# Abolfazlmsl/Oriented-Object-Detection

Measured on AMD Instinct MI355X. Metric: 416px tiles/sec (whole node), YOLOv11n-OBB 3ch, higher is better.
Workload: dtype f32; 1 GPU; YOLOv11n-OBB 3ch 416x416 tiled inference, single-scale (BASELINE configs[1]): forward + decode + ProbIoU NMS + border filter + per-tile merge + final polygon-IoU merge; step_pipelining=True, nc=12, weights=synthetic seeded, cls bias -8 (no checkpoint offline), final_detections=12170

## Files before the change

### include/obbhip.h

```cpp
#ifndef OBBHIP_H
#define OBBHIP_H

#include <stddef.h>
#include <stdint.h>

#ifdef __cplusplus
extern "C" {
#endif

#define OBB_OK 0
#define OBB_ERR_INVALID (-1)
#define OBB_ERR_HIP (-2)
#define OBB_ERR_STATE (-3)
#define OBB_ERR_FORMAT (-4)

typedef struct obb_ctx obb_ctx;
typedef void *obb_stream_t;

int obb_version(void);
int obb_ctx_create(int device, obb_ctx **out);
int obb_ctx_destroy(obb_ctx *ctx);
const char *obb_last_error(const obb_ctx *ctx);

int obb_set_option(obb_ctx *ctx, const char *key, int64_t value);
// ... 110 lines not shown
                      int32_t B, int32_t N, int32_t nh, uint16_t *dqkv, obb_stream_t s);
int obb_add_bf16(obb_ctx *ctx, const uint16_t *a, const uint16_t *b, int64_t n, uint16_t *out, obb_stream_t s);
int obb_chanwin_bf16(obb_ctx *ctx, const uint16_t *src, int32_t Cs, int32_t s0, const uint16_t *add, int32_t Ca, int32_t a0, int64_t npix, int32_t n,
                     uint16_t *dst, int32_t Cd, int32_t d0, obb_stream_t s);

int obb_model_load(obb_ctx *ctx, const void *blob_host, size_t bytes);
int obb_model_unload(obb_ctx *ctx, int32_t slot);
int obb_model_info(const obb_ctx *ctx, int32_t h, int32_t w, int32_t *nc, int32_t *ch, int32_t *anchors, int32_t *nconv);
int obb_forward(obb_ctx *ctx, const uint8_t *tiles, int32_t B, int32_t h, int32_t w, float *head, obb_stream_t s);
int obb_forward_gate(obb_ctx *ctx, const uint8_t *tiles, int32_t B, int32_t h, int32_t w, float *head, float *cmax, obb_stream_t s);
int obb_debug_plan(obb_ctx *ctx, int32_t h, int32_t w, char *buf_host, int64_t buf_bytes, int64_t *needed);
int obb_debug_pack_1x1(int32_t form, const float *w, int32_t cout, int32_t cin, int32_t c0, int32_t nc, float *out, int64_t max_floats,
                       int64_t *needed, int32_t *tiling_host);
int obb_debug_activation(obb_ctx *ctx, int32_t h, int32_t w, int32_t B, const char *name, float *out, int64_t max_elems,
                         int64_t *n_elems, int32_t *shape_hwc_host, obb_stream_t s);
int obb_decode_nms(obb_ctx *ctx, const float *head, int32_t B, int32_t h, int32_t w, float conf_thres, float iou_thres,
                   int32_t max_det, float *out, int32_t *count, obb_stream_t s);
int obb_decode_nms_gate(obb_ctx *ctx, const float *head, const float *cmax, int32_t B, int32_t h, int32_t w, float conf_thres, float iou_thres,
                        int32_t max_det, float *det, int32_t *count, obb_stream_t s);
int obb_decode_nms_full(obb_ctx *ctx, const float *head, int32_t B, int32_t h, int32_t w, float conf_thres, float iou_thres,
                        int32_t max_det, float *out, int32_t *count, obb_stream_t s);
int obb_decode(obb_ctx *ctx, const float *head, int32_t B, int32_t h, int32_t w, float *pred, obb_stream_t s);
int obb_probiou_nms(obb_ctx *ctx, const float *boxes, const float *scores, int64_t n, float iou_thres, int32_t *order,
                    uint8_t *keep, obb_stream_t s);
int obb_results(obb_ctx *ctx, const float *det, const float *lb, int64_t n, float *xywhr, float *pts, obb_stream_t s);

int obb_probiou_loss(obb_ctx *ctx, const float *pred, const float *target, const float *weight, int64_t n, float target_scores_sum,
                     float *loss, float *grad_pred, obb_stream_t s);

int obb_tile_labels(obb_ctx *ctx, const double *labels, int64_t n, const int32_t *rects, int32_t ntiles, double min_fraction, uint8_t *mask,
// ... 66 lines not shown
```

### oriented-object-detection_amd/_lib.py

```python
import ctypes as C
import os

_HERE = os.path.dirname(os.path.abspath(__file__))
SO_PATH = os.path.join(_HERE, "libobbhip.so")
if os.environ.get("OBB_LIB"):
    import sys
    SO_PATH = os.environ["OBB_LIB"]
    sys.stderr.write("oriented_object_detection_amd: OBB_LIB is set -- loading the DIAGNOSTIC library %s instead of the product build\n" % SO_PATH)
_lib = None

c_dp, c_fp, c_ip, c_lp, c_bp = (C.POINTER(C.c_double), C.POINTER(C.c_float), C.POINTER(C.c_int32),
                                C.POINTER(C.c_int64), C.POINTER(C.c_uint8))
_V = C.c_void_p

SIGNATURES = {
    "obb_version": [],
    "obb_ctx_create": [C.c_int, C.POINTER(_V)],
    "obb_ctx_destroy": [_V],
    "obb_last_error": [_V],
    "obb_set_option": [_V, C.c_char_p, C.c_int64],
    "obb_poly_iou_pairs": [_V, _V, _V, C.c_int64, _V, _V],
    "obb_poly_iou_matrix": [_V, _V, _V, C.c_int64, _V, _V, C.c_int64, _V, _V],
    "obb_points_in_quads": [_V, _V, _V, C.c_int64, _V, _V, C.c_int64, _V, _V],
    "obb_build_multich": [_V, _V, C.c_int32, C.c_int32, C.c_int32, _V, _V],
# ... 47 lines not shown
    "obb_attn_fwd_bf16": [_V, _V, C.c_int32, C.c_int32, C.c_int32, _V, _V, _V],
    "obb_attn_bwd_bf16": [_V, _V, _V, _V, _V, _V, C.c_int32, C.c_int32, C.c_int32, _V, _V],
    "obb_add_bf16": [_V, _V, _V, C.c_int64, _V, _V],
    "obb_chanwin_bf16": [_V, _V, C.c_int32, C.c_int32, _V, C.c_int32, C.c_int32, C.c_int64, C.c_int32, _V, C.c_int32, C.c_int32, _V],
    "obb_gather_tiles": [_V, _V, C.c_int32, C.c_int32, C.c_int32, _V, C.c_int32, C.c_int32, _V, _V],
    "obb_letterbox": [_V, _V, C.c_int32, C.c_int32, C.c_int32, C.c_int32, C.c_int32, C.c_int32, C.c_int32, C.c_int32, _V,
                      C.c_int32, C.c_int32, _V],
    "obb_model_load": [_V, _V, C.c_size_t],
    "obb_model_unload": [_V, C.c_int32],
    "obb_model_info": [_V, C.c_int32, C.c_int32, c_ip, c_ip, c_ip, c_ip],
    "obb_forward": [_V, _V, C.c_int32, C.c_int32, C.c_int32, _V, _V],
    "obb_forward_gate": [_V, _V, C.c_int32, C.c_int32, C.c_int32, _V, _V, _V],
    "obb_debug_plan": [_V, C.c_int32, C.c_int32, C.c_char_p, C.c_int64, c_lp],
    "obb_debug_pack_1x1": [C.c_int32, _V, C.c_int32, C.c_int32, C.c_int32, C.c_int32, _V, C.c_int64, c_lp, c_ip],
    "obb_debug_activation": [_V, C.c_int32, C.c_int32, C.c_int32, C.c_char_p, _V, C.c_int64, c_lp, c_ip, _V],
    "obb_decode_nms": [_V, _V, C.c_int32, C.c_int32, C.c_int32, C.c_float, C.c_float, C.c_int32, _V, _V, _V],
    "obb_decode_nms_gate": [_V, _V, _V, C.c_int32, C.c_int32, C.c_int32, C.c_float, C.c_float, C.c_int32, _V, _V, _V],
    "obb_decode_nms_full": [_V, _V, C.c_int32, C.c_int32, C.c_int32, C.c_float, C.c_float, C.c_int32, _V, _V, _V],
    "obb_decode": [_V, _V, C.c_int32, C.c_int32, C.c_int32, _V, _V],
    "obb_probiou_nms": [_V, _V, _V, C.c_int64, C.c_float, _V, _V, _V],
    "obb_results": [_V, _V, _V, C.c_int64, _V, _V, _V],
    "obb_probiou_loss": [_V, _V, _V, _V, C.c_int64, C.c_float, _V, _V, _V],
    "obb_tile_labels": [_V, _V, C.c_int64, _V, C.c_int32, C.c_double, _V, _V, _V],
    "obb_dfl_loss": [_V, _V, _V, _V, C.c_int64, C.c_int32, C.c_float, _V, _V, _V],
    "obb_bce_loss": [_V, _V, _V, C.c_int64, C.c_float, _V, _V, _V],
    "obb_crit_decode": [_V, _V, C.c_int32, _V, _V, c_ip, c_ip, C.c_int32, C.c_int32, _V, _V, _V, _V, _V],
    "obb_crit_loss": [_V, _V, C.c_int32, _V, _V, c_ip, c_ip, C.c_int32, C.c_int32, _V, _V, _V, c_fp, _V, _V, _V, _V, _V, _V],
    "obb_sgd_step": [_V, _V, _V, _V, C.c_int64, C.c_float, C.c_float, C.c_float, C.c_int32, C.c_int32, _V],
    "obb_adamw_step": [_V, _V, _V, _V, _V, C.c_int64, C.c_int64, C.c_float, C.c_double, C.c_double, C.c_float, C.c_float, _V],
    "obb_grad_sumsq_partials": [c_lp, C.c_int32, c_lp],
# ... 51 lines not shown
```

### oriented-object-detection_amd/csrc/c3k2f32.h

```cpp
#pragma once
#include <hip/hip_runtime.h>

#include <vector>

#include "conv.h"

namespace obb {

struct C3k2F32Launch {
    TensorRef cat;
    TensorRef out;
    const float *w1 = nullptr, *w2 = nullptr, *wc = nullptr;
    const float *b1 = nullptr, *b2 = nullptr, *bc = nullptr;
    int B = 0, H = 0, W = 0, C = 16, CO = 64;
};

bool c3k2f32_supported(int C, int CO, int H, int W);
std::vector<int> c3k2f32_cout_perm(int CO);
void c3k2f32_tile(int H, int W, int &TH, int &TW);
hipError_t launch_c3k2f32(const C3k2F32Launch &L, hipStream_t st);

}
```

### oriented-object-detection_amd/csrc/c3k2f32.hip

```cpp
#include "c3k2f32.h"
#include "launchcfg.h"

#include <algorithm>

namespace obb {

typedef __attribute__((ext_vector_type(4))) float f32x4;
typedef __attribute__((ext_vector_type(4))) unsigned int u32x4;

struct C3k2Params {
    const float *cat; int64_t cat_bs; int cat_cs, cat_co; unsigned cat_span;
    float *out; int64_t out_bs; int out_cs, out_co, out_blk, out_ps;
    const float *wall, *b1, *b2;
    int H, W, TH, TW, tiles_x, tiles_y;
    float inv_xw, inv_tw2, inv_tw;
};

__device__ __forceinline__ float silu32c(float x) { return x * __builtin_amdgcn_rcpf(1.0f + __expf(-x)); }

constexpr int kC3MaxX = 448, kC3MaxT = 324;

template <int C, int CO>
__global__ __launch_bounds__(512, 4) void k_c3k2_f32(const C3k2Params P) {
    extern __shared__ __attribute__((aligned(16))) char smem[];
    constexpr int NT = 512, CH = C / 2, PSTX = C * 4 + 16, PSTT = CH * 4 + 16;
    constexpr int CPK1 = C / 4, KP1 = 9 * CPK1 / 4, CPK2 = CH / 4, KP2 = (9 * CPK2) / 4, KR2 = (9 * CPK2) % 4, KPC = 3 * C / 16, NFC = CO / 16;
    static_assert((9 * CPK1) % 4 == 0, "conv 1: whole pieces only");
    constexpr int XOFF = 0, TOFF = kC3MaxX * PSTX, W1OFF = TOFF + kC3MaxT * PSTT, W2OFF = W1OFF + KP1 * 1024, WCOFF = W2OFF + KP2 * 1024 + KR2 * 256,
                  BCOFF = WCOFF + NFC * KPC * 1024, NWCH = (BCOFF + CO * 4 - W1OFF) / 16;
    constexpr int F1 = 3, F2 = 2;
    constexpr unsigned NOPIX = 0xffffffffu;
    const int tid = threadIdx.x, lane = tid & 63, wave = __builtin_amdgcn_readfirstlane(tid >> 6), g = lane >> 4, pl = lane & 15;
    const int t = blockIdx.x, tx_i = t % P.tiles_x, r_ = t / P.tiles_x, ty_i = r_ % P.tiles_y, b = r_ / P.tiles_y;
    const int oy0 = ty_i * P.TH, ox0 = tx_i * P.TW;
    const int XW = P.TW + 4, XH = P.TH + 4, TW2 = P.TW + 2, TH2 = P.TH + 2;
    const int npix1 = TH2 * TW2, npix2 = P.TH * P.TW;

    const __amdgpu_buffer_rsrc_t cat_rsrc = __builtin_amdgcn_make_buffer_rsrc((void *)(P.cat + (int64_t)b * P.cat_bs + P.cat_co), 0, (int)P.cat_span, 0x00020000);
    const __amdgpu_buffer_rsrc_t w_rsrc = __builtin_amdgcn_make_buffer_rsrc((void *)P.wall, 0, NWCH * 16, 0x00020000);
    constexpr int MAXLD = (kC3MaxX * CPK1 + NT - 1) / NT, MAXW = (NWCH + NT - 1) / NT;
    u32x4 xr[MAXLD], wr[MAXW];
    const int nchunkX = XH * XW * CPK1;
#pragma unroll
    for (int k = 0; k < MAXLD; ++k) {
        const int idx = tid + k * NT, pix = idx / CPK1, c = idx - pix * CPK1;
        const int iy = (int)(((float)pix + 0.5f) * P.inv_xw), ix = pix - iy * XW;
        const int gy = oy0 - 2 + iy, gx = ox0 - 2 + ix;
        const bool ok = idx < nchunkX && gy >= 0 && gy < P.H && gx >= 0 && gx < P.W;
        xr[k] = __builtin_amdgcn_raw_buffer_load_b128(cat_rsrc, ok ? (unsigned)((((int64_t)gy * P.W + gx) * P.cat_cs + C + c * 4) * 4) : NOPIX, 0, 0);
    }
#pragma unroll
// ... 22 lines not shown
    for (int k = 0; k < MAXW; ++k) {
        const int idx = tid + k * NT;
        if (idx < NWCH) *reinterpret_cast<u32x4 *>(smem + W1OFF + idx * 16) = wr[k];
    }
    __syncthreads();

    {
        int xb[F1];
        bool val[F1];
#pragma unroll
        for (int i = 0; i < F1; ++i) {
            const int f = wave + 8 * i;
            val[i] = f < nfrag1;
            const int p = min(f * 16 + pl, npix1 - 1);
            const int r = (int)(((float)p + 0.5f) * P.inv_tw2), x = p - r * TW2;
            xb[i] = (r * XW + x) * PSTX;
        }
        f32x4 acc[F1];
#pragma unroll
        for (int i = 0; i < F1; ++i) acc[i] = f32x4{0.f, 0.f, 0.f, 0.f};
        for (int piece = 0; piece < KP1; ++piece) {
            const f32x4 w = *reinterpret_cast<const f32x4 *>(smem + W1OFF + piece * 1024 + lane * 16);
            const int q = piece * 4 + g, tap = q / CPK1, c0 = q - tap * CPK1, dy = (tap * 11) >> 5, dx = tap - dy * 3;
            const int off = (dy * XW + dx) * PSTX + c0 * 16;
            f32x4 a[F1];
#pragma unroll
            for (int i = 0; i < F1; ++i) a[i] = *reinterpret_cast<const f32x4 *>(smem + XOFF + xb[i] + off);
#pragma unroll
            for (int s = 0; s < 4; ++s)
#pragma unroll
                for (int i = 0; i < F1; ++i)
                    if (val[i]) acc[i] = __builtin_amdgcn_mfma_f32_16x16x4f32(w[s], a[i][s], acc[i], 0, 0, 0);
        }
        const float4 bv = *reinterpret_cast<const float4 *>(P.b1 + 4 * g);
#pragma unroll
        for (int i = 0; i < F1; ++i) {
            const int p = (wave + 8 * i) * 16 + pl;
            if (!val[i] || p >= npix1 || 4 * g >= CH) continue;
            const int r = (int)(((float)p + 0.5f) * P.inv_tw2), x = p - r * TW2;
            const int gy = oy0 - 1 + r, gx = ox0 - 1 + x;
            const bool inside = gy >= 0 && gy < P.H && gx >= 0 && gx < P.W;
            float4 o = make_float4(0.f, 0.f, 0.f, 0.f);
            if (inside) o = make_float4(silu32c(acc[i][0] + bv.x), silu32c(acc[i][1] + bv.y), silu32c(acc[i][2] + bv.z), silu32c(acc[i][3] + bv.w));
            *reinterpret_cast<float4 *>(smem + TOFF + (r * TW2 + x) * PSTT + g * 16) = o;
        }
    }
    __syncthreads();

    bool val2[F2];
#pragma unroll
    for (int i = 0; i < F2; ++i) val2[i] = wave + 8 * i < nfrag2;
    f32x4 acc2[F2];
#pragma unroll
    for (int i = 0; i < F2; ++i) acc2[i] = f32x4{0.f, 0.f, 0.f, 0.f};
#pragma unroll
    for (int piece = 0; piece < KP2; ++piece) {
        const f32x4 w = *reinterpret_cast<const f32x4 *>(smem + W2OFF + piece * 1024 + lane * 16);
        const int q = piece * 4 + g, tap = q / CPK2, c0 = q - tap * CPK2, dy = (tap * 11) >> 5, dx = tap - dy * 3;
        const int off = (dy * TW2 + dx) * PSTT + c0 * 16;
// ... 51 lines not shown
#pragma unroll
    for (int i = 0; i < F2; ++i) {
        if (!val2[i] || opix[i] < 0) continue;
        const int ca = P.out_co + 16 * g;
        float *op = P.out + (int64_t)b * P.out_bs + (int64_t)opix[i] * P.out_cs + (P.out_blk ? (int64_t)(ca >> 3) * P.out_ps + (ca & 7) : (int64_t)ca);
#pragma unroll
        for (int nf = 0; nf < NFC; ++nf) {
            const float4 bv = *reinterpret_cast<const float4 *>(smem + BCOFF + (nf * 16 + 4 * g) * 4);
            const float4 o = make_float4(silu32c(acc3[i][nf][0] + bv.x), silu32c(acc3[i][nf][1] + bv.y), silu32c(acc3[i][nf][2] + bv.z), silu32c(acc3[i][nf][3] + bv.w));
            float *o4 = P.out_blk ? op + (int64_t)(nf >> 1) * P.out_ps + 4 * (nf & 1) : op + 4 * nf;
            *reinterpret_cast<float4 *>(o4) = o;
        }
    }
}

void c3k2f32_tile(int H, int W, int &TH, int &TW) {
    TW = std::min(W, 52);
    if (W > 52 && W % 52 && W % 2 == 0 && W / 2 <= 52) TW = W / 2;
    int th = 1;
    while (th + 1 <= H && (th + 5) * (TW + 4) <= kC3MaxX && (th + 3) * (TW + 2) <= kC3MaxT && (th + 3) * (TW + 2) <= 24 * 16 && (th + 1) * TW <= 16 * 16) ++th;
    TH = th;
}

bool c3k2f32_supported(int C, int CO, int H, int W) {
    if (C != 16 || CO != 64 || H < 1 || W < 1) return false;
    int TH, TW;
    c3k2f32_tile(H, W, TH, TW);
    return (TH + 4) * (TW + 4) <= kC3MaxX && (TH + 2) * (TW + 2) <= kC3MaxT && (TH + 2) * (TW + 2) <= 24 * 16 && TH * TW <= 16 * 16;
}

std::vector<int> c3k2f32_cout_perm(int CO) {
    std::vector<int> p(CO);
    for (int f = 0; f < CO / 16; ++f)
        for (int r = 0; r < 16; ++r) p[16 * f + r] = 16 * (r >> 2) + 4 * f + (r & 3);
    return p;
}

hipError_t launch_c3k2f32(const C3k2F32Launch &L, hipStream_t st) {
    if (!c3k2f32_supported(L.C, L.CO, L.H, L.W) || L.cat.cpb || (L.cat.cs & 3) || (L.cat.co & 3) || !L.w1 || !L.b1 || !L.b2 || L.B < 1) return hipErrorInvalidValue;
    if (L.out.cpb && !(L.out.cpb == 2 && L.out.cs == 8 && L.out.co % 8 == 0 && L.out.ps > 0)) return hipErrorInvalidValue;
    if (!L.out.cpb && ((L.out.cs | L.out.co) & 3)) return hipErrorInvalidValue;
    C3k2Params P;
    P.cat = (const float *)L.cat.p; P.cat_bs = L.cat.bs; P.cat_cs = L.cat.cs; P.cat_co = L.cat.co;
    const int64_t span = ((int64_t)L.H * L.W * L.cat.cs - L.cat.co) * 4;
    if (span <= 0 || span >= (1ll << 32) - 65536) return hipErrorInvalidValue;
    P.cat_span = (unsigned)span;
    P.out = (float *)L.out.p; P.out_bs = L.out.bs; P.out_cs = L.out.cs; P.out_co = L.out.co; P.out_blk = L.out.cpb ? 1 : 0; P.out_ps = (int)L.out.ps;
    P.wall = L.w1; P.b1 = L.b1; P.b2 = L.b2;
    P.H = L.H; P.W = L.W;
    c3k2f32_tile(L.H, L.W, P.TH, P.TW);
    P.tiles_x = (L.W + P.TW - 1) / P.TW; P.tiles_y = (L.H + P.TH - 1) / P.TH;
    P.inv_xw = 1.0f / (float)(P.TW + 4); P.inv_tw2 = 1.0f / (float)(P.TW + 2); P.inv_tw = 1.0f / (float)P.TW;
    const int64_t ntiles = (int64_t)L.B * P.tiles_y * P.tiles_x;
    if (ntiles >= (1ll << 31)) return hipErrorInvalidValue;
    constexpr int C = 16, CO = 64;
    constexpr size_t lds = (size_t)kC3MaxX * (C * 4 + 16) + (size_t)kC3MaxT * (C / 2 * 4 + 16) + 9 * 1024 + (4 * 1024 + 2 * 256) + (CO / 16) * 3 * 1024 + CO * 4;
    hipError_t e = allow_dyn_lds((const void *)k_c3k2_f32<16, 64>, 80 * 1024);
    if (e != hipSuccess) return e;
    hipLaunchKernelGGL((k_c3k2_f32<16, 64>), dim3((unsigned)ntiles), dim3(512), lds, st, P);
    return hipGetLastError();
}

}
```

### oriented-object-detection_amd/csrc/ctx.h

```cpp
#pragma once
#include <hip/hip_runtime.h>

#include <cstdarg>
#include <cstdint>
#include <cstdio>
#include <map>
#include <memory>
#include <string>
#include <vector>

#include "../../include/obbhip.h"

namespace obb {
struct Model;
struct EngineOpts {
    bool tail = true, tail16 = true, bneck = true, bneck_cv2 = true, c3kimg = true, dwpw = true, upfold = true, stem = true, front = true, pair = true, hmerge = true,
         sppf_fuse = true, attn_mfma = true, xtile = true, nitile = true, nc2 = true, blk32 = true, c3k2f = true, pw32 = true, upacc = true, graph = true;
    int fwd_split = 0 , microbatch = 1024;
};
}

struct obb_ctx {
    int device = 0;
    std::string err;
    struct Slot { void *p = nullptr; size_t bytes = 0; };
    std::vector<Slot> ws;
    std::shared_ptr<obb::Model> model;
    std::map<int, std::shared_ptr<obb::Model>> slots;
    int slot = 0;
    bool opt_f16 = true;
    bool opt_f32 = false;
    obb::EngineOpts opt;
// ... 28 lines not shown
```

### oriented-object-detection_amd/csrc/engine.hip

```cpp
#include <algorithm>
#include <cmath>
#include <cstdlib>
#include <cstring>

#include "plan.h"

namespace obb {

static int ensure_capacity(obb_ctx *ctx, Plan &P, int B) {
    if (B <= P.cap) return OBB_OK;
    int cap = std::max(B, 1);
    int64_t off = 0;
    for (Buf &b : P.bufs) {
        b.off = off;
        if (b.virt) continue;
        off += ((int64_t)cap * b.per_img() * (b.f32 ? 4 : 2) + 255) / 256 * 256;
    }
    void *slab = nullptr;
    OBB_HIP(ctx, hipDeviceSynchronize());
    P.drop_graphs();
    if (P.slab) { (void)hipFree(P.slab); P.slab = nullptr; P.cap = 0; }
    OBB_HIP(ctx, hipMalloc(&slab, (size_t)off + 256));
    P.slab = slab;
    P.cap = cap;
// ... 214 lines not shown
}

__global__ void k_f32_slice_copy(const float *__restrict__ src, int64_t bs, int cs, int co, int C, int64_t npix_per_img, int B, float *__restrict__ dst, int blk) {
    int64_t i = (int64_t)blockIdx.x * 256 + threadIdx.x;
    if (i >= (int64_t)B * npix_per_img * C) return;
    int c = (int)(i % C) + co;
    int64_t pix = (i / C) % npix_per_img;
    int64_t b = i / ((int64_t)C * npix_per_img);
    dst[i] = blk > 0 ? src[b * bs + (int64_t)(c / blk) * npix_per_img * blk + pix * blk + c % blk] : src[b * bs + pix * cs + c];
}

static bool *switch_of(obb_ctx *ctx, const std::string &k) {
    struct { const char *key; bool *flag; } sw[] = {
        {"tail", &ctx->opt.tail}, {"tail16", &ctx->opt.tail16}, {"bneck", &ctx->opt.bneck}, {"bneck_cv2", &ctx->opt.bneck_cv2},
        {"c3kimg", &ctx->opt.c3kimg}, {"dwpw", &ctx->opt.dwpw}, {"upfold", &ctx->opt.upfold}, {"stem", &ctx->opt.stem}, {"front", &ctx->opt.front}, {"pair", &ctx->opt.pair},
        {"hmerge", &ctx->opt.hmerge}, {"sppf_fuse", &ctx->opt.sppf_fuse}, {"attn_mfma", &ctx->opt.attn_mfma}, {"xtile", &ctx->opt.xtile}, {"nitile", &ctx->opt.nitile}, {"nc2", &ctx->opt.nc2}, {"blk32", &ctx->opt.blk32}, {"c3k2f", &ctx->opt.c3k2f}, {"pw32", &ctx->opt.pw32}, {"upacc", &ctx->opt.upacc}, {"graph", &ctx->opt.graph}};
    for (auto &e : sw)
        if (k == e.key) return e.flag;
    return nullptr;
}

}

using namespace obb;

extern "C" {

int obb_model_load(obb_ctx *ctx, const void *blob_host, size_t bytes) {
    OBB_REQUIRE(ctx, ctx && blob_host && bytes > 0, "obb_model_load: bad arguments");
    OBB_HIP(ctx, hipSetDevice(ctx->device));
    OBB_HIP(ctx, hipDeviceSynchronize());
// ... 174 lines not shown
                break;
            }
            case OP_DW: snprintf(line, sizeof line, "dwconv %s c%d out%dx%d macs%.0f\n", op.name.c_str(), op.in.C, op.Ho, op.Wo, op.macs); break;
            case OP_C3KIMG: snprintf(line, sizeof line, "c3kimg %s c%d out%dx%d macs%.0f\n", op.name.c_str(), op.in.C, op.Ho, op.Wo, op.macs); break;
            case OP_DWPW: snprintf(line, sizeof line, "dwpw %s c%d tail%d out%dx%d macs%.0f\n", op.name.c_str(), op.dwpw.cin, op.dwpw.tail_cout, op.Ho, op.Wo, op.macs); break;
            case OP_BNECK: snprintf(line, sizeof line, "bneck %s c%d co%d out%dx%d rows4 macs%.0f\n", op.name.c_str(), op.bneck.C, op.bneck.CO, op.Ho, op.Wo, op.macs); break;
            case OP_SPPF: snprintf(line, sizeof line, "pool %s c%d out%dx%d x3 macs0\n", op.name.c_str(), op.in.C, op.Ho, op.Wo); break;
            case OP_POOL: snprintf(line, sizeof line, "pool %s c%d out%dx%d macs0\n", op.name.c_str(), op.in.C, op.Ho, op.Wo); break;
            case OP_UP: snprintf(line, sizeof line, "upsample %s c%d out%dx%d macs0\n", op.name.c_str(), op.in.C, op.Ho, op.Wo); break;
            case OP_PW32:
                snprintf(line, sizeof line, "pw32 %s k1 s1 cin%d cout%d out%dx%d waves%d raw%d lds%d macs%.0f\n", op.name.c_str(), op.pw32.cin, op.pw32.cout, op.Ho, op.Wo,
                         op.pw32.cin * 256 <= 80 * 1024 ? 8 : 16, op.pw32.raw ? 1 : 0, op.pw32.cin * 256, op.macs);
                break;
            case OP_C3K2F32: {
                int th, tw;
                c3k2f32_tile(op.H, op.W, th, tw);
                snprintf(line, sizeof line, "c3k2f32 %s c%d co%d out%dx%d TH%d TW%d macs%.0f\n", op.name.c_str(), op.c3k2f.C, op.c3k2f.CO, op.Ho, op.Wo, th, tw, op.macs);
                break;
            }
            case OP_STEM32:
                snprintf(line, sizeof line, "stem32 %s k3 s2 cin%d cout%d out%dx%d rows%d macs%.0f\n", op.name.c_str(), op.stem32.cin, op.stem32.cout, op.Ho, op.Wo, 4, op.macs);
                break;
            case OP_STEM:
                snprintf(line, sizeof line, "stem %s k3 s2 cin%d cout%d out%dx%d rows%d macs%.0f\n", op.name.c_str(), op.stem.cin, op.stem.cout, op.Ho, op.Wo, 4, op.macs);
                break;
            case OP_FRONT: snprintf(line, sizeof line, "front %s cin%d out%dx%d macs%.0f\n", op.name.c_str(), op.front.cin, op.Ho, op.Wo, op.macs); break;
            case OP_ATTN: snprintf(line, sizeof line, "attn %s N%d nh%d macs%.0f\n", op.name.c_str(), op.N, op.nh, op.macs); break;
        }
        out += line;
    }
    snprintf(line, sizeof line, "total_macs %.0f bytes_per_img %lld nbufs %zu nops %zu\n", P->macs_per_img, (long long)P->bytes_per_img, P->bufs.size(),
             P->ops.size());
// ... 22 lines not shown
    const int64_t hw = (int64_t)b.H * b.W;
    const int64_t d_bs = b.blk > 0 ? hw * b.blk : b.per_img(), d_ps = b.blk > 0 ? (int64_t)P->cap * hw * b.blk : 0;
    if (b.f32)
        hipLaunchKernelGGL(k_f32_slice_copy, dim3((unsigned)cdiv(n, 256)), dim3(256), 0, (hipStream_t)s, (const float *)b.p, (int64_t)b.per_img(), b.C, sl.co, sl.C, hw,
                           B, out, b.blk32);
    else if (ctx->model->f16)
        hipLaunchKernelGGL(k_half_slice_to_f32<true>, dim3((unsigned)cdiv(n, 256)), dim3(256), 0, (hipStream_t)s, (const bf16_t *)b.p, d_bs, b.C,
                           sl.co, sl.C, hw, B, out, b.blk, d_ps);
    else
        hipLaunchKernelGGL(k_half_slice_to_f32<false>, dim3((unsigned)cdiv(n, 256)), dim3(256), 0, (hipStream_t)s, (const bf16_t *)b.p, d_bs, b.C,
                           sl.co, sl.C, hw, B, out, b.blk, d_ps);
    OBB_LAUNCH_CHECK(ctx);
    return OBB_OK;
}

}
```

### oriented-object-detection_amd/csrc/netplan.hip

```cpp
#include <algorithm>
#include <cmath>
#include <cstring>

#include "plan.h"

namespace obb {

#pragma pack(push, 1)
struct BlobHeader { char magic[4]; uint32_t version, nrec; int32_t nc, ch; float width, depth; int32_t max_ch, reg_max; char scale[8]; };
struct BlobRec { char name[64]; int32_t c1, c2, k, s, g, act; uint64_t w_off, b_off; };
#pragma pack(pop)

int parse_blob(obb_ctx *ctx, Model &M) {
    const size_t n = M.blob.size();
    if (n < sizeof(BlobHeader)) return set_error(ctx, OBB_ERR_FORMAT, "weight blob too small (%zu bytes)", n);
    BlobHeader H;
    memcpy(&H, M.blob.data(), sizeof H);
    if (memcmp(H.magic, "OBBW", 4) != 0 || H.version != 1) return set_error(ctx, OBB_ERR_FORMAT, "bad weight blob magic/version");
    if (H.reg_max != kRegMax) return set_error(ctx, OBB_ERR_FORMAT, "reg_max %d unsupported", H.reg_max);
    if (H.ch != 3 && H.ch != 4) return set_error(ctx, OBB_ERR_FORMAT, "input channels %d unsupported (3 or 4)", H.ch);
    if (H.nc < 1 || H.nc > 1024) return set_error(ctx, OBB_ERR_FORMAT, "nc %d out of range", H.nc);
    M.nc = H.nc; M.ch = H.ch; M.width = H.width; M.depth = H.depth; M.max_ch = H.max_ch;
    M.scale = std::string(H.scale, strnlen(H.scale, 8));
    size_t tbl = sizeof(BlobHeader);
// ... 536 lines not shown
            for (int i = 0; i < n; ++i) {
                Slice src = sub(cat, (1 + i) * c, c), dst = sub(cat, (2 + i) * c, c);
                if (use_c3k) c3k(name + ".m." + std::to_string(i), src, H, W, dst, 2);
                else bottleneck(name + ".m." + std::to_string(i), src, H, W, dst, 0.5);
            }
        }
        conv(name + ".cv2", whole(cat), H, W, out);
    }
    bool c3k2_f32(const std::string &name, int cat, int c, int H, int W, Slice out) {
        if (!M.f32 || !M.o.tail || !M.o.c3k2f || out.buf < 0 || P.bufs[out.buf].virt || P.bufs[cat].blk32 || !c3k2f32_supported(c, out.C, H, W)) return false;
        const ConvRecord *r1 = rec(name + ".m.0.cv1"), *r2 = rec(name + ".m.0.cv2"), *rc = rec(name + ".cv2");
        if (!r1 || !r2 || !rc || err) return false;
        if (!rec_is(r1, 3, c, c / 2) || !rec_is(r2, 3, c / 2, c) || !rec_is(rc, 1, 3 * c, out.C)) return false;
        const std::vector<int> perm = c3k2f32_cout_perm(out.C);
        const Conv32Tiling t1{1, 1, c, 1, 1, 1, 1}, t2{1, 1, c / 2, 1, 1, 1, 1}, tc{1, 1, 3 * c, out.C / 16, 1, 1, 1};
        std::vector<float> wall = pack_conv32_weights(r1->w, c / 2, c, 3, t1, nullptr, false);
        const std::vector<float> w2 = pack_conv32_weights(r2->w, c, c / 2, 3, t2, nullptr, false), wc = pack_conv32_weights(rc->w, out.C, 3 * c, 1, tc, perm.data(), false);
        wall.insert(wall.end(), w2.begin(), w2.end());
        wall.insert(wall.end(), wc.begin(), wc.end());
        for (int i = 0; i < out.C; ++i) wall.push_back(rc->b[perm[i]]);
        if (wall.size() != (size_t)(9 * 256 + 4 * 256 + 2 * 64 + (out.C / 16) * 3 * 256 + out.C)) { err = set_error(ctx, OBB_ERR_STATE, "c3k2 fp32 kernel: weight image has %zu floats", wall.size()); return false; }
        Op op;
        op.type = OP_C3K2F32; op.name = name + ".m.0+" + name + ".cv2"; op.in = sub(cat, 0, 2 * c); op.out = out; op.H = H; op.W = W; op.Ho = H; op.Wo = W;
        C3k2F32Launch &L = op.c3k2f;
        L.H = H; L.W = W; L.C = c; L.CO = out.C;
        L.w1 = upload(wall); L.b1 = bias_padded(r1, nullptr, 64); L.b2 = bias_padded(r2, nullptr, 64);
        op.macs = (double)H * W * (9.0 * c * (c / 2) * 2 + 3.0 * c * out.C);
        emit(op, name + ".cv2", out);
        return true;
    }

    void head_tail(const std::string &conv1, const std::string &conv2, Slice in, int level, int H, int W, int tmp, Slice head_slice) {
        if (tail_ok(conv1, conv2, H, W)) return conv(conv1, in, H, W, head_slice, Slice(), level, nullptr, conv2.c_str());
        conv(conv1, in, H, W, whole(tmp));
        conv(conv2, whole(tmp), H, W, head_slice, Slice(), level);
    }

    int build() {
        const int h = P.h, w = P.w;
        const bool big = M.scale == "m" || M.scale == "l" || M.scale == "x";
// ... 169 lines not shown
```

### oriented-object-detection_amd/ops.py

```python
import ctypes as C
import contextlib
import ctypes as _ct
import os
from typing import List, Optional

import torch

from . import _lib

_ctx = {}
T = torch.Tensor


def ctx(device=None):
    idx = torch.cuda.current_device() if device is None else torch.device(device).index or 0
    if idx not in _ctx:
        h = C.c_void_p()
        _lib.check(_lib.lib().obb_ctx_create(idx, C.byref(h)))
        _ctx[idx] = h
    return _ctx[idx]


def destroy_contexts():
    for h in _ctx.values():
# ... 1093 lines not shown
    if n:
        _O.records_to_dets(rec, n, r, int(strike_cls), gb, c, f, a)
    return gb, c, f, a


def gather_compact(recv):
    r = _chk(recv, torch.int32, "recv")
    world, cap = r.shape[0], r.shape[1] - 1
    out = torch.empty((world * cap, 12), dtype=torch.int32, device=r.device)
    counts = torch.empty(world + 1, dtype=torch.int32, device=r.device)
    _O.gather_compact(r, out, counts)
    return out, counts


PRECISIONS = {"f16": 16, "fp16": 16, "bf16": 1016, "f32": 32, "fp32": 32}
MODEL_OPTIONS = ("fuse", "tail", "tail16", "bneck", "bneck_cv2", "c3kimg", "dwpw", "upfold", "stem", "front", "pair", "hmerge", "sppf_fuse", "attn_mfma", "xtile", "nitile", "nc2", "blk32", "c3k2f", "pw32", "upacc", "graph")


def select_model(slot, device=None):
    _call("obb_set_option", ctx(device), b"model_slot", int(slot))


def get_option(key, device=None):
    v = C.c_int64(0)
    _call("obb_get_option", ctx(device), key.encode(), C.byref(v))
    return v.value


@contextlib.contextmanager
def engine_state(device=None):
    keys = ("precision",) + MODEL_OPTIONS[1:]
# ... 74 lines not shown
    c = ctx(device)
    need = C.c_int64(0)
    _call("obb_debug_plan", c, h, w, None, 0, C.byref(need))
    buf = C.create_string_buffer(need.value)
    _call("obb_debug_plan", c, h, w, buf, need.value, C.byref(need))
    return buf.value.decode().strip().split("\n")


def debug_activation(name, B, h, w, device=None):
    c = ctx(device)
    n = C.c_int64(0)
    shp = (C.c_int32 * 3)()
    _call("obb_debug_activation", c, h, w, B, name.encode(), None, 0, C.byref(n), shp, _stream())
    out = torch.empty((B, shp[0], shp[1], shp[2]), dtype=torch.float32, device=torch.device("cuda", torch.cuda.current_device()))
    _O.debug_activation(name, B, h, w, out)
    return out


def decode(head, h, w):
    hd = _padded_head(_chk(head, torch.float32, "head"))
    B, A, _ = hd.shape
    pred = torch.empty((B, A, 4 + model_info(h, w, hd.device)["nc"] + 1), dtype=torch.float32, device=hd.device)
    _O.decode(hd, h, w, pred)
    return pred


def decode_nms(head, h, w, conf=0.25, iou=0.7, max_det=300, full=False, zero=True, cmax=None):
    hd = _padded_head(_chk(head, torch.float32, "head"))
    B = hd.shape[0]
    det = (torch.zeros if zero or not B else torch.empty)((B, max_det, 7), dtype=torch.float32, device=hd.device)
# ... 462 lines not shown
```

Measured before the change: 33160 tiles/s.

## Compute two output rows per MFMA fragment in fused C3k2 fp32 first conv

The first 3x3 conv in the fused C3k2 block has only 8 output channels, so half of each 16-wide MFMA fragment was padding. A new rows form packs 8 couts x 2 adjacent output rows into the 16 fragment rows, using a 4x3 (12-tap) weight layout, so the number of fragment columns (pixels) in conv1 is roughly halved. It is enabled by default through a new c3k2rows option and requires even tile heights. A debug entry point to compare the block forms is also added. In exchange it does more K steps per fragment (12 taps instead of 9, with zero-padded weights) and may shrink or change the tile height.

```diff
diff --git a/include/obbhip.h b/include/obbhip.h
--- a/include/obbhip.h
+++ b/include/obbhip.h
@@ -148,6 +148,9 @@
                        int64_t *needed, int32_t *tiling_host);
 int obb_debug_activation(obb_ctx *ctx, int32_t h, int32_t w, int32_t B, const char *name, float *out, int64_t max_elems,
                          int64_t *n_elems, int32_t *shape_hwc_host, obb_stream_t s);
+int obb_debug_c3k2_block(obb_ctx *ctx, int32_t form, int32_t B, int32_t H, int32_t W, int32_t C, int32_t CO, const float *w1_host,
+                         const float *b1_host, const float *w2_host, const float *b2_host, const float *wc_host, const float *bc_host, float *cat3,
+                         float *tmp, float *out, obb_stream_t s);
 int obb_decode_nms(obb_ctx *ctx, const float *head, int32_t B, int32_t h, int32_t w, float conf_thres, float iou_thres,
                    int32_t max_det, float *out, int32_t *count, obb_stream_t s);
 int obb_decode_nms_gate(obb_ctx *ctx, const float *head, const float *cmax, int32_t B, int32_t h, int32_t w, float conf_thres, float iou_thres,
diff --git a/oriented-object-detection_amd/_lib.py b/oriented-object-detection_amd/_lib.py
--- a/oriented-object-detection_amd/_lib.py
+++ b/oriented-object-detection_amd/_lib.py
@@ -85,6 +85,7 @@
     "obb_debug_plan": [_V, C.c_int32, C.c_int32, C.c_char_p, C.c_int64, c_lp],
     "obb_debug_pack_1x1": [C.c_int32, _V, C.c_int32, C.c_int32, C.c_int32, C.c_int32, _V, C.c_int64, c_lp, c_ip],
     "obb_debug_activation": [_V, C.c_int32, C.c_int32, C.c_int32, C.c_char_p, _V, C.c_int64, c_lp, c_ip, _V],
+    "obb_debug_c3k2_block": [_V, C.c_int32, C.c_int32, C.c_int32, C.c_int32, C.c_int32, C.c_int32, _V, _V, _V, _V, _V, _V, _V, _V, _V, _V],
     "obb_decode_nms": [_V, _V, C.c_int32, C.c_int32, C.c_int32, C.c_float, C.c_float, C.c_int32, _V, _V, _V],
     "obb_decode_nms_gate": [_V, _V, _V, C.c_int32, C.c_int32, C.c_int32, C.c_float, C.c_float, C.c_int32, _V, _V, _V],
     "obb_decode_nms_full": [_V, _V, C.c_int32, C.c_int32, C.c_int32, C.c_float, C.c_float, C.c_int32, _V, _V, _V],
diff --git a/oriented-object-detection_amd/csrc/c3k2f32.h b/oriented-object-detection_amd/csrc/c3k2f32.h
--- a/oriented-object-detection_amd/csrc/c3k2f32.h
+++ b/oriented-object-detection_amd/csrc/c3k2f32.h
@@ -13,11 +13,13 @@
     const float *w1 = nullptr, *w2 = nullptr, *wc = nullptr;
     const float *b1 = nullptr, *b2 = nullptr, *bc = nullptr;
     int B = 0, H = 0, W = 0, C = 16, CO = 64;
+    bool rows = true;
 };
 
 bool c3k2f32_supported(int C, int CO, int H, int W);
 std::vector<int> c3k2f32_cout_perm(int CO);
-void c3k2f32_tile(int H, int W, int &TH, int &TW);
+void c3k2f32_tile(int H, int W, int &TH, int &TW, bool rows = true);
+std::vector<float> pack_c3k2_rows_weights(const float *w_oihw, int C);
 hipError_t launch_c3k2f32(const C3k2F32Launch &L, hipStream_t st);
 
 }
diff --git a/oriented-object-detection_amd/csrc/c3k2f32.hip b/oriented-object-detection_amd/csrc/c3k2f32.hip
--- a/oriented-object-detection_amd/csrc/c3k2f32.hip
+++ b/oriented-object-detection_amd/csrc/c3k2f32.hip
@@ -20,21 +20,31 @@
 
 constexpr int kC3MaxX = 448, kC3MaxT = 324;
 
-template <int C, int CO>
+template <int C, int CO, bool ROWS>
+struct C3k2Lds {
+    static constexpr int CH = C / 2, PSTX = C * 4 + 16, PSTT = CH * 4 + 16;
+    static constexpr int CPK1 = C / 4, TAPS1 = ROWS ? 12 : 9, KP1 = TAPS1 * CPK1 / 4, CPK2 = CH / 4, KP2 = (9 * CPK2) / 4, KR2 = (9 * CPK2) % 4, KPC = 3 * C / 16, NFC = CO / 16;
+    static constexpr int XOFF = 0, TOFF = kC3MaxX * PSTX, W1OFF = TOFF + kC3MaxT * PSTT, W2OFF = W1OFF + KP1 * 1024, WCOFF = W2OFF + KP2 * 1024 + KR2 * 256,
+                         BCOFF = WCOFF + NFC * KPC * 1024, BYTES = BCOFF + CO * 4, NWCH = (BYTES - W1OFF) / 16;
+    static_assert((TAPS1 * CPK1) % 4 == 0, "conv 1: whole pieces only");
+    static_assert(2 * BYTES <= 160 * 1024, "two workgroups per CU");
+};
+
+template <int C, int CO, bool ROWS>
 __global__ __launch_bounds__(512, 4) void k_c3k2_f32(const C3k2Params P) {
     extern __shared__ __attribute__((aligned(16))) char smem[];
-    constexpr int NT = 512, CH = C / 2, PSTX = C * 4 + 16, PSTT = CH * 4 + 16;
-    constexpr int CPK1 = C / 4, KP1 = 9 * CPK1 / 4, CPK2 = CH / 4, KP2 = (9 * CPK2) / 4, KR2 = (9 * CPK2) % 4, KPC = 3 * C / 16, NFC = CO / 16;
-    static_assert((9 * CPK1) % 4 == 0, "conv 1: whole pieces only");
-    constexpr int XOFF = 0, TOFF = kC3MaxX * PSTX, W1OFF = TOFF + kC3MaxT * PSTT, W2OFF = W1OFF + KP1 * 1024, WCOFF = W2OFF + KP2 * 1024 + KR2 * 256,
-                  BCOFF = WCOFF + NFC * KPC * 1024, NWCH = (BCOFF + CO * 4 - W1OFF) / 16;
-    constexpr int F1 = 3, F2 = 2;
+    using LY = C3k2Lds<C, CO, ROWS>;
+    constexpr int NT = 512, CH = LY::CH, PSTX = LY::PSTX, PSTT = LY::PSTT;
+    constexpr int CPK1 = LY::CPK1, KP1 = LY::KP1, CPK2 = LY::CPK2, KP2 = LY::KP2, KR2 = LY::KR2, KPC = LY::KPC, NFC = LY::NFC;
+    constexpr int XOFF = LY::XOFF, TOFF = LY::TOFF, W1OFF = LY::W1OFF, W2OFF = LY::W2OFF, WCOFF = LY::WCOFF, BCOFF = LY::BCOFF, NWCH = LY::NWCH;
+    static_assert(!ROWS || CH == 8, "rows form: 8 couts x 2 rows fill the fragment");
+    constexpr int F1 = ROWS ? 2 : 3, F2 = 2;
     constexpr unsigned NOPIX = 0xffffffffu;
     const int tid = threadIdx.x, lane = tid & 63, wave = __builtin_amdgcn_readfirstlane(tid >> 6), g = lane >> 4, pl = lane & 15;
     const int t = blockIdx.x, tx_i = t % P.tiles_x, r_ = t / P.tiles_x, ty_i = r_ % P.tiles_y, b = r_ / P.tiles_y;
     const int oy0 = ty_i * P.TH, ox0 = tx_i * P.TW;
     const int XW = P.TW + 4, XH = P.TH + 4, TW2 = P.TW + 2, TH2 = P.TH + 2;
-    const int npix1 = TH2 * TW2, npix2 = P.TH * P.TW;
+    const int npix1 = (ROWS ? TH2 >> 1 : TH2) * TW2, npix2 = P.TH * P.TW;
 
     const __amdgpu_buffer_rsrc_t cat_rsrc = __builtin_amdgcn_make_buffer_rsrc((void *)(P.cat + (int64_t)b * P.cat_bs + P.cat_co), 0, (int)P.cat_span, 0x00020000);
     const __amdgpu_buffer_rsrc_t w_rsrc = __builtin_amdgcn_make_buffer_rsrc((void *)P.wall, 0, NWCH * 16, 0x00020000);
@@ -87,7 +97,7 @@
             val[i] = f < nfrag1;
             const int p = min(f * 16 + pl, npix1 - 1);
             const int r = (int)(((float)p + 0.5f) * P.inv_tw2), x = p - r * TW2;
-            xb[i] = (r * XW + x) * PSTX;
+            xb[i] = ((ROWS ? 2 * r : r) * XW + x) * PSTX;
         }
         f32x4 acc[F1];
 #pragma unroll
@@ -105,17 +115,19 @@
                 for (int i = 0; i < F1; ++i)
                     if (val[i]) acc[i] = __builtin_amdgcn_mfma_f32_16x16x4f32(w[s], a[i][s], acc[i], 0, 0, 0);
         }
-        const float4 bv = *reinterpret_cast<const float4 *>(P.b1 + 4 * g);
+        const int cg = ROWS ? (g & 1) : g, dyr = ROWS ? (g >> 1) : 0;
+        const float4 bv = *reinterpret_cast<const float4 *>(P.b1 + 4 * cg);
 #pragma unroll
         for (int i = 0; i < F1; ++i) {
             const int p = (wave + 8 * i) * 16 + pl;
-            if (!val[i] || p >= npix1 || 4 * g >= CH) continue;
-            const int r = (int)(((float)p + 0.5f) * P.inv_tw2), x = p - r * TW2;
+            if (!val[i] || p >= npix1 || 4 * cg >= CH) continue;
+            const int rp = (int)(((float)p + 0.5f) * P.inv_tw2), x = p - rp * TW2, r = ROWS ? 2 * rp + dyr : rp;
+            if (r >= TH2) continue;
             const int gy = oy0 - 1 + r, gx = ox0 - 1 + x;
             const bool inside = gy >= 0 && gy < P.H && gx >= 0 && gx < P.W;
             float4 o = make_float4(0.f, 0.f, 0.f, 0.f);
             if (inside) o = make_float4(silu32c(acc[i][0] + bv.x), silu32c(acc[i][1] + bv.y), silu32c(acc[i][2] + bv.z), silu32c(acc[i][3] + bv.w));
-            *reinterpret_cast<float4 *>(smem + TOFF + (r * TW2 + x) * PSTT + g * 16) = o;
+            *reinterpret_cast<float4 *>(smem + TOFF + (r * TW2 + x) * PSTT + cg * 16) = o;
         }
     }
     __syncthreads();
@@ -197,19 +209,42 @@
     }
 }
 
-void c3k2f32_tile(int H, int W, int &TH, int &TW) {
+static bool c3k2f32_fits(int TH, int TW, bool rows) {
+    const int cols1 = rows ? (TH + 2) / 2 * (TW + 2) : (TH + 2) * (TW + 2);
+    return (TH + 4) * (TW + 4) <= kC3MaxX && (TH + 2) * (TW + 2) <= kC3MaxT && cols1 <= (rows ? 16 : 24) * 16 && TH * TW <= 16 * 16 && !(rows && (TH & 1));
+}
+
+void c3k2f32_tile(int H, int W, int &TH, int &TW, bool rows) {
     TW = std::min(W, 52);
     if (W > 52 && W % 52 && W % 2 == 0 && W / 2 <= 52) TW = W / 2;
     int th = 1;
-    while (th + 1 <= H && (th + 5) * (TW + 4) <= kC3MaxX && (th + 3) * (TW + 2) <= kC3MaxT && (th + 3) * (TW + 2) <= 24 * 16 && (th + 1) * TW <= 16 * 16) ++th;
+    while (th + 1 <= H && c3k2f32_fits(th + 1, TW, false)) ++th;
+    if (rows && (th & 1)) th = c3k2f32_fits(th + 1, TW, true) ? th + 1 : th - 1;
     TH = th;
 }
 
 bool c3k2f32_supported(int C, int CO, int H, int W) {
     if (C != 16 || CO != 64 || H < 1 || W < 1) return false;
-    int TH, TW;
-    c3k2f32_tile(H, W, TH, TW);
-    return (TH + 4) * (TW + 4) <= kC3MaxX && (TH + 2) * (TW + 2) <= kC3MaxT && (TH + 2) * (TW + 2) <= 24 * 16 && TH * TW <= 16 * 16;
+    for (int rows = 0; rows < 2; ++rows) {
+        int TH, TW;
+        c3k2f32_tile(H, W, TH, TW, rows != 0);
+        if (TH < 1 || !c3k2f32_fits(TH, TW, rows != 0)) return false;
+    }
+    return true;
+}
+
+std::vector<float> pack_c3k2_rows_weights(const float *w, int C) {
+    const int CH = C / 2, cpk = C / 4;
+    std::vector<float> out((size_t)12 * cpk / 4 * 256, 0.f);
+    size_t o = 0;
+    for (int piece = 0; piece < 12 * cpk / 4; ++piece)
+        for (int lane = 0; lane < 64; ++lane)
+            for (int s = 0; s < 4; ++s, ++o) {
+                const int q = piece * 4 + (lane >> 4), tap = q / cpk, c = (q % cpk) * 4 + s, wy = tap / 3, wx = tap % 3;
+                const int r = lane & 15, co = r % CH, dy = r / CH, ky = wy - dy;
+                if (dy < 2 && ky >= 0 && ky < 3) out[o] = w[((size_t)co * C + c) * 9 + ky * 3 + wx];
+            }
+    return out;
 }
 
 std::vector<int> c3k2f32_cout_perm(int CO) {
@@ -231,16 +266,22 @@
     P.out = (float *)L.out.p; P.out_bs = L.out.bs; P.out_cs = L.out.cs; P.out_co = L.out.co; P.out_blk = L.out.cpb ? 1 : 0; P.out_ps = (int)L.out.ps;
     P.wall = L.w1; P.b1 = L.b1; P.b2 = L.b2;
     P.H = L.H; P.W = L.W;
-    c3k2f32_tile(L.H, L.W, P.TH, P.TW);
+    c3k2f32_tile(L.H, L.W, P.TH, P.TW, L.rows);
+    if (!c3k2f32_fits(P.TH, P.TW, L.rows)) return hipErrorInvalidValue;
     P.tiles_x = (L.W + P.TW - 1) / P.TW; P.tiles_y = (L.H + P.TH - 1) / P.TH;
     P.inv_xw = 1.0f / (float)(P.TW + 4); P.inv_tw2 = 1.0f / (float)(P.TW + 2); P.inv_tw = 1.0f / (float)P.TW;
     const int64_t ntiles = (int64_t)L.B * P.tiles_y * P.tiles_x;
     if (ntiles >= (1ll << 31)) return hipErrorInvalidValue;
-    constexpr int C = 16, CO = 64;
-    constexpr size_t lds = (size_t)kC3MaxX * (C * 4 + 16) + (size_t)kC3MaxT * (C / 2 * 4 + 16) + 9 * 1024 + (4 * 1024 + 2 * 256) + (CO / 16) * 3 * 1024 + CO * 4;
-    hipError_t e = allow_dyn_lds((const void *)k_c3k2_f32<16, 64>, 80 * 1024);
-    if (e != hipSuccess) return e;
-    hipLaunchKernelGGL((k_c3k2_f32<16, 64>), dim3((unsigned)ntiles), dim3(512), lds, st, P);
+    constexpr size_t lds_rows = C3k2Lds<16, 64, true>::BYTES, lds_one = C3k2Lds<16, 64, false>::BYTES;
+    if (L.rows) {
+        hipError_t e = allow_dyn_lds((const void *)k_c3k2_f32<16, 64, true>, 80 * 1024);
+        if (e != hipSuccess) return e;
+        hipLaunchKernelGGL((k_c3k2_f32<16, 64, true>), dim3((unsigned)ntiles), dim3(512), lds_rows, st, P);
+    } else {
+        hipError_t e = allow_dyn_lds((const void *)k_c3k2_f32<16, 64, false>, 80 * 1024);
+        if (e != hipSuccess) return e;
+        hipLaunchKernelGGL((k_c3k2_f32<16, 64, false>), dim3((unsigned)ntiles), dim3(512), lds_one, st, P);
+    }
     return hipGetLastError();
 }
 
diff --git a/oriented-object-detection_amd/csrc/ctx.h b/oriented-object-detection_amd/csrc/ctx.h
--- a/oriented-object-detection_amd/csrc/ctx.h
+++ b/oriented-object-detection_amd/csrc/ctx.h
@@ -15,7 +15,7 @@
 struct Model;
 struct EngineOpts {
     bool tail = true, tail16 = true, bneck = true, bneck_cv2 = true, c3kimg = true, dwpw = true, upfold = true, stem = true, front = true, pair = true, hmerge = true,
-         sppf_fuse = true, attn_mfma = true, xtile = true, nitile = true, nc2 = true, blk32 = true, c3k2f = true, pw32 = true, upacc = true, graph = true;
+         sppf_fuse = true, attn_mfma = true, xtile = true, nitile = true, nc2 = true, blk32 = true, c3k2f = true, c3k2rows = true, pw32 = true, upacc = true, graph = true;
     int fwd_split = 0 , microbatch = 1024;
 };
 }
diff --git a/oriented-object-detection_amd/csrc/engine.hip b/oriented-object-detection_amd/csrc/engine.hip
--- a/oriented-object-detection_amd/csrc/engine.hip
+++ b/oriented-object-detection_amd/csrc/engine.hip
@@ -252,7 +252,7 @@
     struct { const char *key; bool *flag; } sw[] = {
         {"tail", &ctx->opt.tail}, {"tail16", &ctx->opt.tail16}, {"bneck", &ctx->opt.bneck}, {"bneck_cv2", &ctx->opt.bneck_cv2},
         {"c3kimg", &ctx->opt.c3kimg}, {"dwpw", &ctx->opt.dwpw}, {"upfold", &ctx->opt.upfold}, {"stem", &ctx->opt.stem}, {"front", &ctx->opt.front}, {"pair", &ctx->opt.pair},
-        {"hmerge", &ctx->opt.hmerge}, {"sppf_fuse", &ctx->opt.sppf_fuse}, {"attn_mfma", &ctx->opt.attn_mfma}, {"xtile", &ctx->opt.xtile}, {"nitile", &ctx->opt.nitile}, {"nc2", &ctx->opt.nc2}, {"blk32", &ctx->opt.blk32}, {"c3k2f", &ctx->opt.c3k2f}, {"pw32", &ctx->opt.pw32}, {"upacc", &ctx->opt.upacc}, {"graph", &ctx->opt.graph}};
+        {"hmerge", &ctx->opt.hmerge}, {"sppf_fuse", &ctx->opt.sppf_fuse}, {"attn_mfma", &ctx->opt.attn_mfma}, {"xtile", &ctx->opt.xtile}, {"nitile", &ctx->opt.nitile}, {"nc2", &ctx->opt.nc2}, {"blk32", &ctx->opt.blk32}, {"c3k2f", &ctx->opt.c3k2f}, {"c3k2rows", &ctx->opt.c3k2rows}, {"pw32", &ctx->opt.pw32}, {"upacc", &ctx->opt.upacc}, {"graph", &ctx->opt.graph}};
     for (auto &e : sw)
         if (k == e.key) return e.flag;
     return nullptr;
@@ -457,8 +457,9 @@
                 break;
             case OP_C3K2F32: {
                 int th, tw;
-                c3k2f32_tile(op.H, op.W, th, tw);
-                snprintf(line, sizeof line, "c3k2f32 %s c%d co%d out%dx%d TH%d TW%d macs%.0f\n", op.name.c_str(), op.c3k2f.C, op.c3k2f.CO, op.Ho, op.Wo, th, tw, op.macs);
+                c3k2f32_tile(op.H, op.W, th, tw, op.c3k2f.rows);
+                snprintf(line, sizeof line, "c3k2f32 %s c%d co%d out%dx%d TH%d TW%d rows%d macs%.0f\n", op.name.c_str(), op.c3k2f.C, op.c3k2f.CO, op.Ho, op.Wo, th, tw,
+                         op.c3k2f.rows ? 2 : 1, op.macs);
                 break;
             }
             case OP_STEM32:
@@ -511,4 +512,64 @@
     return OBB_OK;
 }
 
-}
+int obb_debug_c3k2_block(obb_ctx *ctx, int32_t form, int32_t B, int32_t H, int32_t W, int32_t C, int32_t CO, const float *w1, const float *b1,
+                         const float *w2, const float *b2, const float *wc, const float *bc, float *cat3, float *tmp, float *out, obb_stream_t s) {
+    OBB_REQUIRE(ctx, ctx && w1 && b1 && w2 && b2 && wc && bc && cat3 && out && (form != 0 || tmp), "obb_debug_c3k2_block: bad arguments");
+    OBB_REQUIRE(ctx, form >= 0 && form <= 2 && B >= 1 && H >= 1 && W >= 1 && C >= 16 && C % 16 == 0 && CO >= 16 && CO % 16 == 0 && (int64_t)B * H * W * 3 * C < (1ll << 30),
+                "obb_debug_c3k2_block: bad shape");
+    OBB_REQUIRE(ctx, form == 0 || c3k2f32_supported(C, CO, H, W), "obb_debug_c3k2_block: no block kernel for C %d CO %d at %d x %d", C, CO, H, W);
+    OBB_HIP(ctx, hipSetDevice(ctx->device));
+    hipStream_t st = (hipStream_t)s;
+    std::vector<void *> held;
+    hipError_t e = hipSuccess;
+    auto upload = [&](const std::vector<float> &v) -> const float * {
+        void *p = nullptr;
+        if (e == hipSuccess) e = hipMalloc(&p, v.size() * 4);
+        if (e == hipSuccess) { held.push_back(p); e = hipMemcpy(p, v.data(), v.size() * 4, hipMemcpyHostToDevice); }
+        return (const float *)p;
+    };
+    auto padded = [&](const float *b, int n) { std::vector<float> v((n + 63) / 64 * 64, 0.f); std::copy(b, b + n, v.begin()); return v; };
+    auto slice = [&](float *p, int cs, int co) { TensorRef t; t.p = p; t.bs = (int64_t)H * W * cs; t.cs = cs; t.co = co; return t; };
+    if (form == 0) {
+        auto conv = [&](int ks, int cin, int cout, const float *w, const float *b, TensorRef in, TensorRef o, TensorRef res) {
+            Conv32Launch L;
+            const Conv32Tiling t = plan_conv32(ks, 1, cin, cout, H, W, false, false, ctx->opt.nc2);
+            L.ks = ks; L.stride = 1; L.cin = cin; L.cout = cout; L.act = 1;
+            L.set_tiling(t); L.NC = std::max(1, t.NC);
+            L.B = B; L.Hin = L.Hout = H; L.Win = L.Wout = W;
+            L.tiles_y = (H + t.TH - 1) / t.TH; L.tiles_x = (W + t.TW - 1) / t.TW;
+            if (ks == 1) {
+                const int64_t npx = (int64_t)B * H * W;
+                L.B = 1; L.Hin = L.Hout = 1; L.Win = L.Wout = (int)npx; L.tiles_y = 1; L.tiles_x = (int)((npx + t.TW - 1) / t.TW);
+            }
+            L.wpk = upload(pack_conv32_weights(w, cout, cin, ks, t, nullptr, false));
+            L.bias = upload(padded(b, cout));
+            L.in = in; L.out = o; L.res = res; L.xtile = ctx->opt.xtile;
+            if (e == hipSuccess) e = launch_conv32(L, st);
+        };
+        conv(3, C, C / 2, w1, b1, slice(cat3, 3 * C, C), slice(tmp, C / 2, 0), TensorRef());
+        conv(3, C / 2, C, w2, b2, slice(tmp, C / 2, 0), slice(cat3, 3 * C, 2 * C), slice(cat3, 3 * C, C));
+        conv(1, 3 * C, CO, wc, bc, slice(cat3, 3 * C, 0), slice(out, CO, 0), TensorRef());
+    } else {
+        const bool rows = form == 2;
+        const std::vector<int> perm = c3k2f32_cout_perm(CO);
+        const Conv32Tiling t1{1, 1, C, 1, 1, 1, 1}, t2{1, 1, C / 2, 1, 1, 1, 1}, tc{1, 1, 3 * C, CO / 16, 1, 1, 1};
+        std::vector<float> wall = rows ? pack_c3k2_rows_weights(w1, C) : pack_conv32_weights(w1, C / 2, C, 3, t1, nullptr, false);
+        const std::vector<float> p2 = pack_conv32_weights(w2, C, C / 2, 3, t2, nullptr, false), pc = pack_conv32_weights(wc, CO, 3 * C, 1, tc, perm.data(), false);
+        wall.insert(wall.end(), p2.begin(), p2.end());
+        wall.insert(wall.end(), pc.begin(), pc.end());
+        for (int i = 0; i < CO; ++i) wall.push_back(bc[perm[i]]);
+        C3k2F32Launch L;
+        L.B = B; L.H = H; L.W = W; L.C = C; L.CO = CO; L.rows = rows;
+        L.cat = slice(cat3, 3 * C, 0); L.out = slice(out, CO, 0);
+        L.w1 = upload(wall); L.b1 = upload(padded(b1, C / 2)); L.b2 = upload(padded(b2, C));
+        if (e == hipSuccess) e = launch_c3k2f32(L, st);
+    }
+    const hipError_t es = hipStreamSynchronize(st);
+    for (void *p : held) (void)hipFree(p);
+    OBB_HIP(ctx, e);
+    OBB_HIP(ctx, es);
+    return OBB_OK;
+}
+
+}
diff --git a/oriented-object-detection_amd/csrc/netplan.hip b/oriented-object-detection_amd/csrc/netplan.hip
--- a/oriented-object-detection_amd/csrc/netplan.hip
+++ b/oriented-object-detection_amd/csrc/netplan.hip
@@ -574,16 +574,17 @@
         if (!rec_is(r1, 3, c, c / 2) || !rec_is(r2, 3, c / 2, c) || !rec_is(rc, 1, 3 * c, out.C)) return false;
         const std::vector<int> perm = c3k2f32_cout_perm(out.C);
         const Conv32Tiling t1{1, 1, c, 1, 1, 1, 1}, t2{1, 1, c / 2, 1, 1, 1, 1}, tc{1, 1, 3 * c, out.C / 16, 1, 1, 1};
-        std::vector<float> wall = pack_conv32_weights(r1->w, c / 2, c, 3, t1, nullptr, false);
+        const bool rows = M.o.c3k2rows;
+        std::vector<float> wall = rows ? pack_c3k2_rows_weights(r1->w, c) : pack_conv32_weights(r1->w, c / 2, c, 3, t1, nullptr, false);
         const std::vector<float> w2 = pack_conv32_weights(r2->w, c, c / 2, 3, t2, nullptr, false), wc = pack_conv32_weights(rc->w, out.C, 3 * c, 1, tc, perm.data(), false);
         wall.insert(wall.end(), w2.begin(), w2.end());
         wall.insert(wall.end(), wc.begin(), wc.end());
         for (int i = 0; i < out.C; ++i) wall.push_back(rc->b[perm[i]]);
-        if (wall.size() != (size_t)(9 * 256 + 4 * 256 + 2 * 64 + (out.C / 16) * 3 * 256 + out.C)) { err = set_error(ctx, OBB_ERR_STATE, "c3k2 fp32 kernel: weight image has %zu floats", wall.size()); return false; }
+        if (wall.size() != (size_t)((rows ? 12 : 9) * 256 + 4 * 256 + 2 * 64 + (out.C / 16) * 3 * 256 + out.C)) { err = set_error(ctx, OBB_ERR_STATE, "c3k2 fp32 kernel: weight image has %zu floats", wall.size()); return false; }
         Op op;
         op.type = OP_C3K2F32; op.name = name + ".m.0+" + name + ".cv2"; op.in = sub(cat, 0, 2 * c); op.out = out; op.H = H; op.W = W; op.Ho = H; op.Wo = W;
         C3k2F32Launch &L = op.c3k2f;
-        L.H = H; L.W = W; L.C = c; L.CO = out.C;
+        L.H = H; L.W = W; L.C = c; L.CO = out.C; L.rows = rows;
         L.w1 = upload(wall); L.b1 = bias_padded(r1, nullptr, 64); L.b2 = bias_padded(r2, nullptr, 64);
         op.macs = (double)H * W * (9.0 * c * (c / 2) * 2 + 3.0 * c * out.C);
         emit(op, name + ".cv2", out);
diff --git a/oriented-object-detection_amd/ops.py b/oriented-object-detection_amd/ops.py
--- a/oriented-object-detection_amd/ops.py
+++ b/oriented-object-detection_amd/ops.py
@@ -1131,7 +1131,7 @@
 
 
 PRECISIONS = {"f16": 16, "fp16": 16, "bf16": 1016, "f32": 32, "fp32": 32}
-MODEL_OPTIONS = ("fuse", "tail", "tail16", "bneck", "bneck_cv2", "c3kimg", "dwpw", "upfold", "stem", "front", "pair", "hmerge", "sppf_fuse", "attn_mfma", "xtile", "nitile", "nc2", "blk32", "c3k2f", "pw32", "upacc", "graph")
+MODEL_OPTIONS = ("fuse", "tail", "tail16", "bneck", "bneck_cv2", "c3kimg", "dwpw", "upfold", "stem", "front", "pair", "hmerge", "sppf_fuse", "attn_mfma", "xtile", "nitile", "nc2", "blk32", "c3k2f", "c3k2rows", "pw32", "upacc", "graph")
 
 
 def select_model(slot, device=None):
@@ -1236,6 +1236,25 @@
     _call("obb_debug_activation", c, h, w, B, name.encode(), None, 0, C.byref(n), shp, _stream())
     out = torch.empty((B, shp[0], shp[1], shp[2]), dtype=torch.float32, device=torch.device("cuda", torch.cuda.current_device()))
     _O.debug_activation(name, B, h, w, out)
+    return out
+
+
+def debug_c3k2_block(cat, w1, b1, w2, b2, wc, bc, form=2):
+    import numpy as np
+    t = _chk(cat, torch.float32, "cat")
+    B, H, W, C2 = t.shape
+    Cn, CO = C2 // 2, int(wc.shape[0])
+    host = [np.ascontiguousarray(np.asarray(v, dtype=np.float32)) for v in (w1, b1, w2, b2, wc, bc)]
+    if host[0].shape != (Cn // 2, Cn, 3, 3) or host[2].shape != (Cn, Cn // 2, 3, 3) or host[4].reshape(CO, -1).shape != (CO, 3 * Cn) or \
+            [v.size for v in host[1::2]] != [Cn // 2, Cn, CO]:
+        raise ValueError("debug_c3k2_block: weight shapes do not match a C3k2 block of %d channels" % Cn)
+    cat3 = torch.zeros((B, H, W, 3 * Cn), dtype=torch.float32, device=t.device)
+    cat3[..., :C2] = t
+    tmp = torch.empty((B, H, W, Cn // 2), dtype=torch.float32, device=t.device)
+    out = torch.empty((B, H, W, CO), dtype=torch.float32, device=t.device)
+    torch.cuda.current_stream().synchronize()
+    _call("obb_debug_c3k2_block", ctx(t.device), int(form), B, H, W, Cn, CO, *[C.c_void_p(v.ctypes.data) for v in host], _p(cat3), _p(tmp), _p(out),
+          _stream())
     return out
 
 
```

New measurement: 33360 tiles/s (median of 6 runs). No clear change (+0.6%).
